# VisualComputingInstitute/diffusion-e2e-ft

Measured on AMD Instinct MI355X. Metric: images/sec (768x768, 1-step UNet fwd) full path: VAE encode + SD-v2 UNet @t=999 + VAE decode, higher is better.
Workload: dtype f16

## Files before the change

### diffusion-e2e-ft_amd/_lib.py

```python
import ctypes as C
import os

import torch

from . import build as _build

_LIB = None

F32, F16, BF16 = 0, 1, 2
_DT = {torch.float32: F32, torch.float16: F16, torch.bfloat16: BF16}


def dtype_id(dt):
    try:
        return _DT[dt]
    except KeyError:
        raise TypeError("libe2eft supports float32/float16/bfloat16, got %s" % dt)


class ConvDesc(C.Structure):
    _fields_ = [(n, C.c_int32) for n in (
        "dtype", "batch", "hin", "win", "hl", "wl", "c1", "ldx1", "c2", "ldx2", "kh", "kw", "stride", "pad_t", "pad_l",
        "hout", "wout", "cout", "ldo", "ldr", "ldw")] + [("alpha", C.c_float)]


class GemmDesc(C.Structure):
    _fields_ = ([(n, C.c_int32) for n in ("dtype", "m", "n", "k", "lda", "ldw", "ldo", "ldr", "nzo", "nzi")]
                + [(n, C.c_int64) for n in ("sa_o", "sa_i", "sw_o", "sw_i", "so_o", "so_i", "sr_o", "sr_i")]
                + [("bias_along_m", C.c_int32), ("alpha", C.c_float)])


class GroupNormDesc(C.Structure):
    _fields_ = [(n, C.c_int32) for n in ("dtype", "batch", "hw", "c1", "ldx1", "c2", "ldx2", "groups", "ldy", "silu")] + [
        ("eps", C.c_float)]


class AttnDesc(C.Structure):
    _fields_ = [(n, C.c_int32) for n in ("dtype", "batch", "heads", "nq", "nk_seg", "kv_nseg", "kv_bmod", "ldq", "ldk", "ldv",
                                          "ldo")] + [("scale", C.c_float)]


class NormalEvalDesc(C.Structure):
    _fields_ = [(n, C.c_int32) for n in ("batch", "height", "width", "reserved")] + [
        ("pred_stride", C.c_int64 * 4), ("gt_stride", C.c_int64 * 4), ("mask_stride", C.c_int64 * 3)]


class D2ntDesc(C.Structure):
    _fields_ = [(n, C.c_int32) for n in ("batch", "height", "width", "refine", "out_format")] + [("depth_scale", C.c_float)]


D2NT_F32, D2NT_U16, D2NT_U8 = range(3)


class HypersimDesc(C.Structure):
    _fields_ = [(n, C.c_int32) for n in ("batch", "height", "width", "color_dtype", "distance_dtype", "depth_format")] + [
        ("focal", C.c_double), ("scale_numerator", C.c_double)]


HYPERSIM_DEPTH_U16, HYPERSIM_DEPTH_F32 = range(2)
HYPERSIM_RECORD = 16


class DepthGtDesc(C.Structure):
    _fields_ = ([(n, C.c_int32) for n in ("batch", "h0", "w0", "raw_dtype")] + [("divisor", C.c_double)]
                + [(n, C.c_int32) for n in ("inf_to_zero", "crop_top", "crop_left", "crop_h", "crop_w")] + [("min_depth", C.c_float), ("max_depth", C.c_float)]
                + [(n, C.c_int32) for n in ("win_y0", "win_y1", "win_x0", "win_x1", "use_ext_mask")])


GT_U16, GT_I32, GT_F32 = range(3)


class NormalGtDesc(C.Structure):
    _fields_ = [(n, C.c_int32) for n in ("batch", "height", "width", "raw_dtype")]


NORMAL_GT_U8, NORMAL_GT_F32 = range(2)


class DsineRgbDesc(C.Structure):
    _fields_ = [(n, C.c_int32) for n in ("batch", "height", "width", "out_layout")]


class DiffusionDesc(C.Structure):
    _fields_ = [(n, C.c_int32) for n in ("dtype", "dtype_out", "prediction", "rows", "hw", "c", "batch", "ldx0", "ldn", "ldy", "n_timesteps")]


DIFFUSION_ADD_NOISE, DIFFUSION_VELOCITY = range(2)
PREDICTION_TYPES = {"epsilon": 0, "v_prediction": 1}


RGB_HWC, RGB_CHW = range(2)
DSINE_RGB_WS_INTS = 6


OPT_PERSISTENT, OPT_PERSISTENT_GRID, OPT_NARROW_CONV, OPT_NARROW_MFMA, OPT_IGEMM_GENERAL_OPERANDS, OPT_IGEMM2_WAVES, OPT_PATCH_CONV, OPT_THIN_INPUT_CONV, OPT_FUSED_NORM, OPT_ATTN_DMA, OPT_UPCONV_PHASES, OPT_PATCH_CONV_2X2, OPT_PERSISTENT_MIN_QROUNDS, OPT_GN_APPLY_ITERS, OPT_F32_SPLIT, OPT_F32_SPLIT_ATTN, OPT_PATCH_MFMA = range(17)

_P = C.c_void_p
_I = C.c_int32
_L = C.c_int64
_F = C.c_float
_Z = C.c_size_t

SIGNATURES = {
    "e2eft_version": (_I, []),
    "e2eft_last_error": (C.c_char_p, []),
    "e2eft_build_id": (C.c_char_p, []),
    "e2eft_set_option": (_I, [_I, _I]),
    "e2eft_get_option": (_I, [_I]),
    "e2eft_conv2d_fwd": (_I, [C.POINTER(ConvDesc), _P, _P, _P, _P, _P, _P, _P, _P]),
    "e2eft_gemm": (_I, [C.POINTER(GemmDesc), _P, _P, _P, _P, _P, _P]),
    "e2eft_conv2d_fwd_gnstats": (_I, [C.POINTER(ConvDesc), _P, _P, _P, _P, _P, _P, _P, _P, _Z, C.POINTER(C.c_int32), _P]),
    "e2eft_conv2d_splitk_workspace_bytes": (_Z, [C.POINTER(ConvDesc)]),
    "e2eft_conv2d_fwd_splitk": (_I, [C.POINTER(ConvDesc), _P, _P, _P, _P, _P, _P, _P, _P, _Z, _P]),
    "e2eft_gemm_gnstats": (_I, [C.POINTER(GemmDesc), _P, _P, _P, _P, _P, _I, _P, _Z, C.POINTER(C.c_int32), _P]),
    "e2eft_groupnorm_fwd_pre": (_I, [C.POINTER(GroupNormDesc), _P, _P, _P, _P, _P, _P, _I, _P, _I, _P, _Z, _P]),
    "e2eft_groupnorm_coeff_offset": (_Z, [C.POINTER(GroupNormDesc)]),
    "e2eft_groupnorm_fwd_stats": (_I, [C.POINTER(GroupNormDesc), _P, _P, _P, _P, _I, _P, _I, _P, _Z, _P]),
    "e2eft_conv2d_fwd_normed_supported": (_I, [C.POINTER(ConvDesc)]),
    "e2eft_upconv2x_fwd_supported": (_I, [C.POINTER(ConvDesc)]),
    "e2eft_upconv2x_fwd": (_I, [C.POINTER(ConvDesc), _P, _P, _P, _P, _P, _Z, C.POINTER(C.c_int32), _P]),
    "e2eft_groupnorm_fwd_split": (_I, [C.POINTER(GroupNormDesc), _P, _P, _P, _P, _I, _P, _P, _I, _P, _Z, _P]),
    "e2eft_f32_split_weight": (_I, [_P, _L, _I, _P, _P, _P]),
    "e2eft_f32_split2_cat": (_I, [_P, _I, _I, _P, _I, _I, _L, _P, _I, _P, _P]),
    "e2eft_f32_split2": (_I, [_P, _L, _I, _I, _P, _I, _P, _P]),
    "e2eft_f32_split2_cols": (_I, [_P, _I, _I, _P, _I, _I, _L, _P, _I, _P, _P]),
    "e2eft_f32_split_wgrad_finish": (_I, [_P, _P, _P, _L, _I, _I, _P, _P, _P, _P]),
    "e2eft_conv2d_fwd_f32split_supported": (_I, [C.POINTER(ConvDesc)]),
    "e2eft_conv2d_fwd_f32split": (_I, [C.POINTER(ConvDesc), _P, _P, _P, _P, _P, _P, _P, _P, _Z, C.POINTER(C.c_int32), _P]),
    "e2eft_upconv2x_fwd_f32split_supported": (_I, [C.POINTER(ConvDesc)]),
    "e2eft_upconv2x_fwd_f32split": (_I, [C.POINTER(ConvDesc), _P, _P, _P, _P, _P, _P, _P, _Z, C.POINTER(C.c_int32), _P]),
    "e2eft_gemm_f32split_supported": (_I, [C.POINTER(GemmDesc)]),
    "e2eft_attn_f32split_supported": (_I, [C.POINTER(AttnDesc), _I]),
    "e2eft_gemm_f32split": (_I, [C.POINTER(GemmDesc), _P, _P, _P, _P, _P, _P, _P, _P]),
    "e2eft_conv2d_fwd_normed": (_I, [C.POINTER(ConvDesc), _P, _P, _P, _I, _P, _P, _P, _P, _P, _P, _Z, C.POINTER(C.c_int32), _P]),
    "e2eft_groupnorm_workspace_bytes": (_Z, [C.POINTER(GroupNormDesc)]),
    "e2eft_groupnorm_fwd": (_I, [C.POINTER(GroupNormDesc), _P, _P, _P, _P, _P, _P, _Z, _P]),
    "e2eft_layernorm_fwd": (_I, [_I, _L, _I, _I, _I, _F, _P, _P, _P, _P, _P]),
    "e2eft_geglu_fwd": (_I, [_I, _L, _I, _I, _I, _P, _P, _P]),
    "e2eft_softmax_rows": (_I, [_I, _L, _I, _L, _F, _P, _P]),
    "e2eft_softmax_rows_causal": (_I, [_I, _L, _I, _L, _F, _I, _P, _P]),
    "e2eft_attn_fwd": (_I, [C.POINTER(AttnDesc), _P, _P, _P, _P, _P]),
    "e2eft_attn_fwd_lse": (_I, [C.POINTER(AttnDesc), _P, _P, _P, _P, _P, _P]),
    "e2eft_attn512_workspace_bytes": (_Z, [C.POINTER(AttnDesc)]),
    "e2eft_attn512_fwd": (_I, [C.POINTER(AttnDesc), _P, _P, _P, _P, _P, _Z, _P]),
    "e2eft_attn_bwd_workspace_bytes": (_Z, [C.POINTER(AttnDesc)]),
    "e2eft_attn_bwd": (_I, [C.POINTER(AttnDesc), _P, _P, _P, _P, _P, _I, _P, _P, _I, _P, _I, _P, _I, _P, _Z, _P]),
    "e2eft_nchw_to_nhwc": (_I, [_I, _I, _I, _I, _I, _I, _I, _F, _F, _P, _P, _P]),
    "e2eft_nhwc_to_nchw": (_I, [_I, _I, _I, _I, _I, _I, _F, _F, _P, _P, _P]),
    "e2eft_copy_scale": (_I, [_I, _L, _I, _I, _I, _F, _F, _P, _P, _P]),
    "e2eft_add": (_I, [_I, _L, _I, _I, _I, _I, _P, _P, _P, _P]),
    "e2eft_timestep_embedding": (_I, [_I, _I, _I, _P, _P, _P]),
    "e2eft_silu": (_I, [_I, _L, _P, _P, _P]),
    "e2eft_depth_head": (_I, [_I, _I, _L, _I, _I, _P, _P, _P]),
    "e2eft_normal_head": (_I, [_I, _I, _I, _I, _I, _I, _F, _P, _P, _P]),
    "e2eft_ssi_loss_workspace_bytes": (_Z, [_I]),
    "e2eft_ssi_loss_fwd": (_I, [_I, _I, _P, _P, _P, _P, _P, _P, _Z, _P]),
    "e2eft_angular_loss_workspace_bytes": (_Z, [_I]),
    "e2eft_angular_loss_fwd": (_I, [_I, _I, _P, _P, _P, _P, _P, _Z, _P]),
    "e2eft_conv2d_dgrad": (_I, [C.POINTER(ConvDesc), _P, _I, _I, _P, _I, _P, _I, _P]),
    "e2eft_conv2d_wgrad_workspace_bytes": (_Z, [C.POINTER(ConvDesc), _I]),
    "e2eft_conv2d_wgrad": (_I, [C.POINTER(ConvDesc), _P, _I, _P, _P, _P, _Z, C.POINTER(C.c_int32), _P]),
    "e2eft_conv2d_im2col_t": (_I, [C.POINTER(ConvDesc), _P, _P, _P, _L, _P]),
    "e2eft_transpose": (_I, [_I, _I, _L, _I, _L, _L, _L, _L, _L, _P, _P, _P]),
    "e2eft_colsum_workspace_bytes": (_Z, [_I, _L, _I]),
    "e2eft_colsum": (_I, [_I, _I, _L, _I, _L, _F, _P, _P, _P, _Z, _P]),
    "e2eft_upsample_nearest_bwd": (_I, [_I, _I, _I, _I, _I, _I, _I, _I, _I, _P, _P, _P]),
    "e2eft_groupnorm_bwd_workspace_bytes": (_Z, [C.POINTER(GroupNormDesc)]),
    "e2eft_groupnorm_bwd": (_I, [C.POINTER(GroupNormDesc), _P, _P, _P, _P, _P, _I, _P, _I, _P, _P, _P, _P, _Z, _P]),
    "e2eft_groupnorm_bwd_add": (_I, [C.POINTER(GroupNormDesc), _P, _P, _P, _P, _P, _I, _P, _I, _P, _I, _P, _P, _P, _P, _Z, _P]),
    "e2eft_layernorm_bwd_workspace_bytes": (_Z, [_L, _I]),
    "e2eft_layernorm_bwd": (_I, [_I, _L, _I, _I, _I, _I, _F, _P, _P, _P, _P, _P, _P, _Z, _P]),
    "e2eft_geglu_bwd": (_I, [_I, _L, _I, _I, _I, _I, _P, _P, _P, _P]),
    "e2eft_softmax_bwd_rows": (_I, [_I, _L, _I, _L, _F, _P, _P, _P]),
    "e2eft_silu_bwd": (_I, [_I, _L, _P, _P, _P, _P]),
    "e2eft_depth_head_bwd": (_I, [_I, _I, _L, _I, _I, _I, _I, _P, _P, _P, _P]),
    "e2eft_normal_head_bwd": (_I, [_I, _I, _I, _I, _I, _I, _I, _I, _F, _P, _P, _P, _P]),
    "e2eft_ssi_loss_bwd_workspace_bytes": (_Z, [_I]),
    "e2eft_ssi_loss_bwd": (_I, [_I, _I, _P, _P, _P, _P, _P, _P, _P, _P, _Z, _P]),
# ... 118 lines not shown
```

### diffusion-e2e-ft_amd/csrc/api.hip

```cpp
#include "common.h"
#include <atomic>

namespace e2eft {

static thread_local char g_err[512] = "";

char* err_buf() { return g_err; }

int fail(int code, const char* fmt, ...) {
    va_list ap;
    va_start(ap, fmt);
    vsnprintf(g_err, sizeof(g_err), fmt, ap);
    va_end(ap);
    return code;
}

int check_launch(const char* what) {
    hipError_t e = hipGetLastError();
    if (e != hipSuccess) return fail(E2EFT_ERR_LAUNCH, "%s: launch failed: %s", what, hipGetErrorString(e));
    return E2EFT_OK;
}

static std::atomic<int> g_cus_of_device[64];
int device_cus() {
    int dev = 0;
    if (hipGetDevice(&dev) != hipSuccess || dev < 0 || dev >= 64) return 0;
    int n = g_cus_of_device[dev].load(std::memory_order_relaxed);
    if (n == 0) {
        if (hipDeviceGetAttribute(&n, hipDeviceAttributeMultiprocessorCount, dev) != hipSuccess || n < 8) return 0;
        n &= ~7;
        g_cus_of_device[dev].store(n, std::memory_order_relaxed);
    }
    return n;
}

static thread_local char g_tag[96] = "";
void tag_kernel(const char* fmt, ...) {
    va_list ap;
    va_start(ap, fmt);
    vsnprintf(g_tag, sizeof(g_tag), fmt, ap);
    va_end(ap);
}
const char* last_tag() { return g_tag; }

static std::atomic<int> g_opt[E2EFT_OPT_COUNT] = {{1}, {0}, {1}, {1}, {0}, {0}, {1}, {1}, {1}, {1}, {1}, {1}, {2}, {0}, {1}, {0}, {0}};

int option(int key) { return g_opt[key].load(std::memory_order_relaxed); }

}

extern "C" int e2eft_set_option(int32_t key, int32_t value) {
    using namespace e2eft;
    E2EFT_REQUIRE(key >= 0 && key < E2EFT_OPT_COUNT, "set_option: unknown key %d", key);
    bool ok = value == 0 || value == 1;
    if (key == E2EFT_OPT_PERSISTENT_GRID) ok = value == 0 || (value >= 8 && value % 8 == 0 && value <= 4096);
    if (key == E2EFT_OPT_IGEMM2_WAVES) ok = value == 0 || value == 4 || value == 8;
    if (key == E2EFT_OPT_PERSISTENT_MIN_QROUNDS) ok = value >= 1 && value <= 64;
    if (key == E2EFT_OPT_GN_APPLY_ITERS) ok = value >= 0 && value <= 16;
    if (key == E2EFT_OPT_PATCH_MFMA) ok = value >= 0 && value <= 2;
    E2EFT_REQUIRE(ok, "set_option: value %d out of range for key %d", value, key);
    g_opt[key].store(value, std::memory_order_relaxed);
    return E2EFT_OK;
}
extern "C" int e2eft_get_option(int32_t key) { return key >= 0 && key < E2EFT_OPT_COUNT ? e2eft::option(key) : -1; }

extern "C" const char* e2eft_debug_last_kernel(void) { return e2eft::last_tag(); }

extern "C" int e2eft_version(void) { return E2EFT_VERSION; }
#ifndef E2EFT_BUILD_ID
#define E2EFT_BUILD_ID "unstamped"
#endif
static const char k_build_id[] = "E2EFT_BUILD_ID=" E2EFT_BUILD_ID;
extern "C" const char* e2eft_build_id(void) { return k_build_id + 15; }
extern "C" const char* e2eft_last_error(void) { return e2eft::err_buf(); }
```

### diffusion-e2e-ft_amd/csrc/igemm5.hip

```cpp
#include "igemm.h"
#include <atomic>
#include <type_traits>

namespace e2eft {

namespace pers {
constexpr int BM = 256, BN = 128, NW = 8;
constexpr int A_STAGE = BM * 128, B_STAGE = BN * 128, STAGE = A_STAGE + B_STAGE;
constexpr int RING = 3 * STAGE;
constexpr int DEP = NW * 64 * 3 * 4;
constexpr int ROWTAB = BM * 16;
constexpr int LDS = RING + DEP + ROWTAB;
}

#ifdef E2EFT_STAMPS
static __device__ long long g_stamps5[512 * 32 * 8];
#define STAMP5(t, i) do { if (threadIdx.x == 0 && (t) < 32 && blockIdx.x < 512) g_stamps5[(blockIdx.x * 32 + (t)) * 8 + (i)] = __builtin_readcyclecounter(); } while (0)
#else
#define STAMP5(t, i) do { } while (0)
#endif

template <typename T, int MODE, bool RES, bool F32O = false>
__global__ __launch_bounds__(512) void igemm5_kernel(const IgemmParams p, const int total_tiles) {
    using namespace pers;
    static_assert(!F32O || (RES && std::is_same<T, f16>::value), "fp32 output: the fp32-window epilogue, f16 split operands");
    __shared__ __attribute__((aligned(16))) char smem[LDS];
    constexpr int EPC = 8;
    constexpr int BK = 64;
    constexpr int RSTEP = 8 * NW;
    typedef float f2 __attribute__((ext_vector_type(2)));

    const int tid = threadIdx.x;
    const int lane = tid & 63;
    const int wave = __builtin_amdgcn_readfirstlane(tid >> 6);
    const int wm = wave >> 1, wn = wave & 1;
    const int l31 = lane & 31, h = lane >> 5;
    const int nblk = p.mtiles * p.ntiles;
    const int nk = p.K / BK;

    const int nslots = (int)gridDim.x >> 3, xcd = (int)blockIdx.x & 7, slot = (int)blockIdx.x >> 3;
    const int q8 = total_tiles >> 3, r8 = total_tiles & 7;
    const int cbeg = xcd < r8 ? xcd * (q8 + 1) : r8 * (q8 + 1) + (xcd - r8) * q8;
    const int cend = cbeg + (xcd < r8 ? q8 + 1 : q8);
    int u_dma = cbeg + slot;
    if (u_dma >= cend) return;

    const int lrow = 8 * wave + (lane >> 3);
    const int jc = (lane & 7) ^ ((lrow >> 1) & 7);
    const bool plain_taps = MODE == 1 && p.zins <= 1 && p.hl == p.hin && p.wl == p.win;
    const bool half_res = MODE == 1 && (p.zins == 2 || (p.zins <= 1 && p.hl == 2 * p.hin && p.wl == 2 * p.win));

    unsigned int off1[4], off2[4];
    unsigned int cur_a[4], cur_b[2];
    unsigned int base1[4], base2[4];
    int a_iy0[4], a_ix0[4], brel[4];
    int tile_c = 0, ky = 0, kx = 0;
    int d_m0 = 0, d_n0 = 0, d_zo = 0, d_zi = 0;
    bool dma_done = false;
    __amdgpu_buffer_rsrc_t rs1, rs2, rsw, rsa;

    int d_b0 = 0;
    auto tile_coords = [&](const int u) {
        int z = 0, lid = u;
        if (nblk != total_tiles) { z = fast_div(u, nblk); lid = u - z * nblk; }
        int mt = lid, nt = 0;
        if (p.ntiles > 1) { mt = fast_div(lid, p.ntiles); nt = lid - mt * p.ntiles; }
        d_m0 = mt * BM; d_n0 = nt * BN;
        d_zo = 0; d_zi = z;
        if (p.nzi > 1 && z > 0) { d_zo = fast_div(z, p.nzi); d_zi = z - d_zo * p.nzi; }
        else if (p.nzi == 1) { d_zo = z; d_zi = 0; }
        if (MODE == 1) d_b0 = fast_div(d_m0, p.hout * p.wout);
    };
    auto fill_rowtab = [&]() {
        if (MODE == 1 && tid < BM) {
            const int hw = p.hout * p.wout;
            const int m = d_m0 + tid;
            const int b = fast_div(m, hw);
            const int rem = m - b * hw;
            const int oy = fast_div(rem, p.wout), ox = rem - oy * p.wout;
            int iy0 = oy * p.stride - p.pad_t, ix0 = ox * p.stride - p.pad_l;
            if (F32O && m >= p.M) iy0 = -0x4000;
            const u32x4 v = {(unsigned)(b - d_b0), (unsigned)iy0, (unsigned)ix0, (unsigned)(((b - d_b0) * p.hin + iy0) * p.win + ix0)};
            const unsigned addr = (unsigned)(RING + DEP) + (unsigned)tid * 16u;
            asm volatile("ds_write_b128 %0, %1" :: "v"(addr), "v"(v) : "memory");
        }
    };
    auto finish_setup = [&]() {
        const T* X1 = (const T*)p.x1 + d_zo * p.sa_o + d_zi * p.sa_i;
        const T* W = (const T*)p.w + d_zo * p.sw_o + d_zi * p.sw_i;
        const T* b1;
        const T* b2 = (const T*)p.x2;
        if (MODE == 0) {
            b1 = X1 + (long)d_m0 * p.ldx1;
#pragma unroll
            for (int i = 0; i < 4; ++i) cur_a[i] = ((F32O && d_m0 + lrow + RSTEP * i >= p.M) ? SRD_OOB : (unsigned)((lrow + RSTEP * i) * p.ldx1 + jc * EPC) * (unsigned)sizeof(T)) - 128u;
        } else {
            b1 = X1 + (long)d_b0 * p.hin * p.win * p.ldx1;
            if (b2) b2 += (long)d_b0 * p.hin * p.win * p.ldx2;
            u32x4 rt[4];
#pragma unroll
            for (int i = 0; i < 4; ++i) {
                const unsigned addr = (unsigned)(RING + DEP) + (unsigned)(lrow + RSTEP * i) * 16u;
                asm volatile("ds_read_b128 %0, %1" : "=v"(rt[i]) : "v"(addr) : "memory");
            }
            asm volatile("s_waitcnt lgkmcnt(0)" : "+v"(rt[0]), "+v"(rt[1]), "+v"(rt[2]), "+v"(rt[3]) :: "memory");
#pragma unroll
            for (int i = 0; i < 4; ++i) {
                brel[i] = (int)rt[i][0]; a_iy0[i] = (int)rt[i][1]; a_ix0[i] = (int)rt[i][2];
                cur_a[i] = 0;
                if (plain_taps) {
                    base1[i] = (rt[i][3] * (unsigned)p.ldx1 + (unsigned)(jc * EPC)) * (unsigned)sizeof(T);
                    base2[i] = (rt[i][3] * (unsigned)p.ldx2 + (unsigned)(jc * EPC)) * (unsigned)sizeof(T);
                }
            }
        }
        rs1 = whole_range_rsrc(b1);
        rs2 = whole_range_rsrc((b2 ? b2 : b1));
        rsw = whole_range_rsrc((W + (long)d_n0 * p.ldw));
        rsa = rs1;
// ... 26 lines not shown
                off1[i] = ok ? (pix * (unsigned)p.ldx1 + (unsigned)(jc * EPC)) * (unsigned)sizeof(T) : SRD_OOB;
                off2[i] = ok ? (pix * (unsigned)p.ldx2 + (unsigned)(jc * EPC)) * (unsigned)sizeof(T) : SRD_OOB;
            }
            return;
        }
#pragma unroll
        for (int i = 0; i < 4; ++i) {
            const int iy = a_iy0[i] + ky, ix = a_ix0[i] + kx;
            bool ok = (unsigned)iy < (unsigned)p.hl && (unsigned)ix < (unsigned)p.wl;
            int sy = iy, sx = ix;
            if (p.zins > 1) {
                ok = ok && (iy % p.zins == 0) && (ix % p.zins == 0);
                sy = iy / p.zins; sx = ix / p.zins;
            } else {
                if (p.hl != p.hin) sy = min((int)floorf(iy * p.up_sh), p.hin - 1);
                if (p.wl != p.win) sx = min((int)floorf(ix * p.up_sw), p.win - 1);
            }
            const unsigned pix = (unsigned)((brel[i] * p.hin + sy) * p.win + sx);
            off1[i] = ok ? (pix * (unsigned)p.ldx1 + (unsigned)(jc * EPC)) * (unsigned)sizeof(T) : SRD_OOB;
            off2[i] = ok ? (pix * (unsigned)p.ldx2 + (unsigned)(jc * EPC)) * (unsigned)sizeof(T) : SRD_OOB;
        }
    };
#ifdef E2EFT_STAMPS
    bool fire_a = true;
#endif
    auto advance = [&]() {
#ifdef E2EFT_STAMPS
        fire_a = !(p.debug_flags & 1) && !((p.debug_flags & 2) && kx != 0) && !((p.debug_flags & 4) && (kx != 0 || ky != 0));
#endif
        if (MODE == 0) {
            if constexpr (F32O) {
                const unsigned back = tile_c == p.split_c ? (unsigned)p.split_c * 2u : 0u;
                tile_c += BK;
#pragma unroll
                for (int i = 0; i < 4; ++i) cur_a[i] += 128u - back;
            } else {
#pragma unroll
                for (int i = 0; i < 4; ++i) cur_a[i] += 128u;
            }
        } else {
            if (F32O && tile_c == p.split_c) {
#pragma unroll
                for (int i = 0; i < 4; ++i) cur_a[i] = off1[i];
            } else if (tile_c == 0) {
                retap();
#pragma unroll
                for (int i = 0; i < 4; ++i) cur_a[i] = off1[i];
                rsa = rs1;
            } else if (tile_c == p.c1) {
#pragma unroll
                for (int i = 0; i < 4; ++i) cur_a[i] = off2[i];
                rsa = rs2;
            } else {
#pragma unroll
                for (int i = 0; i < 4; ++i) cur_a[i] += 128u;
            }
            tile_c += BK;
            if (tile_c >= p.cin) {
                tile_c = 0;
                if (++kx == p.kw) { kx = 0; ++ky; }
            }
        }
        cur_b[0] += 128u;
        cur_b[1] += 128u;
    };
    int s_cur = 0, s_nxt = STAGE, s_dst = 2 * STAGE;
    auto rotate = [&]() { const int t = s_cur; s_cur = s_nxt; s_nxt = s_dst; s_dst = t; };
    auto fire = [&](const int stage, auto piece_c) {
        constexpr int Q = decltype(piece_c)::value;
        char* sa = smem + stage + wave * 1024;
#ifdef E2EFT_STAMPS
        if (Q < 4 && !fire_a) return;
#endif
        if constexpr (Q < 4) __builtin_amdgcn_raw_ptr_buffer_load_lds(rsa, (lds_ptr_t)(sa + Q * (RSTEP * 128)), 16, cur_a[Q], 0, 0, 0);
        else __builtin_amdgcn_raw_ptr_buffer_load_lds(rsw, (lds_ptr_t)(sa + A_STAGE + (Q - 4) * (RSTEP * 128)), 16, cur_b[Q - 4], 0, 0, 0);
    };
    auto fire_all = [&](const int stage) {
        fire(stage, IConst<0>{}); fire(stage, IConst<1>{}); fire(stage, IConst<2>{}); fire(stage, IConst<3>{});
        fire(stage, IConst<4>{}); fire(stage, IConst<5>{});
    };

    int tseq = 0;
    (void)tseq;
    floatx16 acc[2][2];
    const int sw = (l31 >> 1) & 7;
    int aofs[4], bofs[4];
#pragma unroll
    for (int g = 0; g < 4; ++g) {
        const int chunk = g * 2 + h;
        aofs[g] = (wm * 64 + l31) * 128 + ((chunk ^ sw) * 16);
        bofs[g] = A_STAGE + (wn * 64 + l31) * 128 + ((chunk ^ sw) * 16);
    }
    auto mma_group = [&](const u32x4& a0, const u32x4& a1, const u32x4& b0, const u32x4& b1) {
        acc[0][0] = Mma32x32x16<T>::run(a0, b0, acc[0][0]);
        acc[0][1] = Mma32x32x16<T>::run(a0, b1, acc[0][1]);
        acc[1][0] = Mma32x32x16<T>::run(a1, b0, acc[1][0]);
        acc[1][1] = Mma32x32x16<T>::run(a1, b1, acc[1][1]);
    };

    const int er = lane >> 3, ec = lane & 7;
    const T* __restrict__ bias = (const T*)p.bias;
    const T* __restrict__ rowadd = (const T*)p.rowadd;
    constexpr bool has_res = RES && !F32O;
    const bool has_ra = rowadd != nullptr, stats = p.gn_partial != nullptr;
    Vec16<T> pre_res[4], pre_bias, pre_ra;
    T col_bias[2], col_ra[2];
    long c_orow = 0, c_rrow = 0;
    int c_m0 = 0, c_n0 = 0, c_img = 0, c_ncl = 0;
    int c_mb = 0, c_seg0 = 0;
    bool c_colok = false;

    const int npre = F32O ? 0 : has_res ? 4 + (bias ? 1 : 0) + (has_ra ? 1 : 0) : 2 * ((bias ? 1 : 0) + (has_ra ? 1 : 0));
    bool nxt = false;
    long zoff_o = 0;
    auto enter_tile = [&]() {
        c_m0 = d_m0; c_n0 = d_n0;
        zoff_o = d_zo * p.so_o + d_zi * p.so_i;
        const long zoff_r = d_zo * p.sr_o + d_zi * p.sr_i;
        c_colok = c_n0 + wn * 64 + ec * 8 < p.N;
        c_ncl = c_colok ? c_n0 + wn * 64 + ec * 8 : c_n0;
        c_img = has_ra ? fast_div(c_m0, p.rows_per_img) : 0;
        const int m = c_m0 + wm * 64 + er;
        c_mb = c_m0 + wm * 64;
        c_seg0 = p.out_seg > 0 ? fast_div(c_mb, p.out_seg) : 0;
        c_orow = ((long)m + (long)c_seg0 * p.out_seg) * p.ldo + c_ncl;
        c_rrow = zoff_r + (long)m * p.ldr + c_ncl;
        nxt = u_dma + nslots < cend;
        if (nxt) tile_coords(u_dma + nslots);
    };
    auto ktile = [&](auto kind_c, const int nextwait) {
        constexpr int KIND = decltype(kind_c)::value;
        if (KIND == 0 || KIND == 3 || (KIND == 2 && !dma_done)) advance();
        const int sc = s_cur, sd = s_dst;
        u32x4 a0[3], a1[3], b0[3], b1[3];
        auto rd = [&](auto gc, auto slotc) {
            constexpr int g = decltype(gc)::value, slot = decltype(slotc)::value;
            a0[slot] = *reinterpret_cast<const u32x4*>(smem + sc + aofs[g]);
            a1[slot] = *reinterpret_cast<const u32x4*>(smem + sc + aofs[g] + 32 * 128);
            b0[slot] = *reinterpret_cast<const u32x4*>(smem + sc + bofs[g]);
            b1[slot] = *reinterpret_cast<const u32x4*>(smem + sc + bofs[g] + 32 * 128);
        };
        rd(IConst<0>{}, IConst<0>{});
        rd(IConst<1>{}, IConst<1>{});
        __builtin_amdgcn_sched_barrier(0);
        rd(IConst<2>{}, IConst<2>{});
        if constexpr (KIND != 1) { fire(sd, IConst<0>{}); fire(sd, IConst<1>{}); }
        __builtin_amdgcn_sched_barrier(0);
        if constexpr (KIND == 3) {
            const floatx16 z = {0.f, 0.f, 0.f, 0.f, 0.f, 0.f, 0.f, 0.f, 0.f, 0.f, 0.f, 0.f, 0.f, 0.f, 0.f, 0.f};
            acc[0][0] = Mma32x32x16<T>::run(a0[0], b0[0], z);
            acc[0][1] = Mma32x32x16<T>::run(a0[0], b1[0], z);
            acc[1][0] = Mma32x32x16<T>::run(a1[0], b0[0], z);
            acc[1][1] = Mma32x32x16<T>::run(a1[0], b1[0], z);
        } else {
            mma_group(a0[0], a1[0], b0[0], b1[0]);
        }
        __builtin_amdgcn_sched_barrier(0);
        if constexpr (KIND == 3) enter_tile();
        if constexpr (KIND == 1) {
            if constexpr (F32O) {
            } else if (has_res) {
#pragma unroll
                for (int s = 0; s < 4; ++s) pre_res[s] = ld16((const T*)p.residual + c_rrow + (long)(s * 8) * p.ldr);
                if (bias) pre_bias = ld16(bias + c_ncl);
                if (has_ra) pre_ra = ld16(rowadd + (long)c_img * p.N + c_ncl);
            } else {
                const int cA = c_n0 + wn * 64 + l31, cB = cA + 32;
                const int nA = cA < p.N ? cA : c_n0, nB = cB < p.N ? cB : c_n0;
                if (bias) { col_bias[0] = bias[nA]; col_bias[1] = bias[nB]; }
                if (has_ra) { col_ra[0] = rowadd[(long)c_img * p.N + nA]; col_ra[1] = rowadd[(long)c_img * p.N + nB]; }
            }
            u_dma += nslots;
            if (nxt) {
                finish_setup();
                advance();
            } else {
                dma_done = true;
#pragma unroll
                for (int i = 0; i < 4; ++i) cur_a[i] = SRD_OOB;
                cur_b[0] = cur_b[1] = SRD_OOB;
            }
            __builtin_amdgcn_sched_barrier(0);
            fire(sd, IConst<0>{}); fire(sd, IConst<1>{});
        }
        rd(IConst<3>{}, IConst<0>{});
        fire(sd, IConst<2>{}); fire(sd, IConst<3>{});
        __builtin_amdgcn_sched_barrier(0);
        mma_group(a0[1], a1[1], b0[1], b1[1]);
        __builtin_amdgcn_sched_barrier(0);
        fire(sd, IConst<4>{}); fire(sd, IConst<5>{});
        if constexpr (KIND == 3) {
            if (nxt) fill_rowtab();
        }
        __builtin_amdgcn_sched_barrier(0);
        if (nextwait == 2) asm volatile("s_waitcnt vmcnt(6) lgkmcnt(0)" ::: "memory");
        else if (nextwait == 3) {
            if (npre == 0) asm volatile("s_waitcnt vmcnt(6) lgkmcnt(0)" ::: "memory");
            else if (npre == 1) asm volatile("s_waitcnt vmcnt(7) lgkmcnt(0)" ::: "memory");
            else if (npre == 2) asm volatile("s_waitcnt vmcnt(8) lgkmcnt(0)" ::: "memory");
            else if (npre == 4) asm volatile("s_waitcnt vmcnt(10) lgkmcnt(0)" ::: "memory");
            else if (npre == 5) asm volatile("s_waitcnt vmcnt(11) lgkmcnt(0)" ::: "memory");
            else asm volatile("s_waitcnt vmcnt(12) lgkmcnt(0)" ::: "memory");
        } else asm volatile("s_waitcnt lgkmcnt(0)" ::: "memory");
        __builtin_amdgcn_s_barrier();
        asm volatile("" ::: "memory");
        __builtin_amdgcn_sched_barrier(0);
        mma_group(a0[2], a1[2], b0[2], b1[2]);
        mma_group(a0[0], a1[0], b0[0], b1[0]);
        asm volatile("" ::: "memory");
        rotate();
    };

    auto epi_rows_left = [&]() -> int { return F32O ? p.M - (c_m0 + wm * 64 + er) : 0x40000000; };
    auto epi_rofs = [&](const int r) -> long {
        if (p.out_seg <= 0) return (long)r;
        return (long)r + (long)(fast_div(c_mb + r, p.out_seg) - c_seg0) * p.out_seg;
    };
    constexpr int EPI_DEP = RING;
    constexpr bool EPI_M16 = false;
    auto epi_srow = [&](const int s) -> int { return 8 * s; };
#define EPI_STAMP(i) STAMP5(tseq, i)
#include "igemm_persistent_epilogue.inc"
#undef EPI_STAMP
    const float al_f32 = F32O ? p.alpha * (p.alpha_dev ? *p.alpha_dev : 1.f) * (p.alpha_dev2 ? *p.alpha_dev2 : 1.f) : 0.f;
    tile_coords(u_dma);
    fill_rowtab();
    __syncthreads();
    finish_setup();
    advance(); fire_all(s_cur);
    advance(); fire_all(s_nxt);
    asm volatile("s_waitcnt vmcnt(6)" ::: "memory");
    __builtin_amdgcn_s_barrier();
    asm volatile("" ::: "memory");
    bool first = true;
    for (;;) {
        STAMP5(tseq, 0);
        ktile(IConst<3>{}, first ? 2 : 0);
        for (int kt = 1; kt < nk - 2; ++kt) ktile(IConst<0>{}, 2);
        STAMP5(tseq, 1);
        ktile(IConst<1>{}, 3);
        STAMP5(tseq, 4);
        ktile(IConst<2>{}, 0);
        STAMP5(tseq, 2);
        if constexpr (F32O) epilogue_f32(s_dst, al_f32);
        else if constexpr (RES) epilogue(s_dst, zoff_o);
        else epilogue_packed(s_dst, zoff_o);
        STAMP5(tseq, 3);
        ++tseq;
        asm volatile("s_waitcnt lgkmcnt(0)" ::: "memory");
        __builtin_amdgcn_s_barrier();
        asm volatile("" ::: "memory");
        if (stats) { const int img = c_m0 / p.rows_per_img; combine(img, (c_m0 - img * p.rows_per_img) / BM, c_n0); }
        STAMP5(tseq - 1, 7);
        if (dma_done) break;
        first = false;
    }
}

static std::atomic<long> g_pers_launches{0};

#ifdef E2EFT_STAMPS
extern int g_debug_flags5;
#endif

template <typename T, int MODE> static int launch5(IgemmParams& p, int nz, int total, int grid, hipStream_t s) {
    if constexpr (std::is_same<T, f16>::value) {
        if (p.split_c > 0) {
            hipLaunchKernelGGL((igemm5_kernel<f16, MODE, true, true>), dim3(grid), dim3(512), 0, s, p, total);
            tag_kernel("igemm5_kernel<_Float16, %d, true, f32split>", MODE);
            return check_launch("igemm5");
        }
    }
    if (p.residual) hipLaunchKernelGGL((igemm5_kernel<T, MODE, true>), dim3(grid), dim3(512), 0, s, p, total);
    else hipLaunchKernelGGL((igemm5_kernel<T, MODE, false>), dim3(grid), dim3(512), 0, s, p, total);
    tag_kernel("igemm5_kernel<%s, %d, %s>", std::is_same<T, f16>::value ? "_Float16" : "__bf16", MODE, p.residual ? "true" : "false");
    return check_launch("igemm5");
}

bool igemm_persistent_eligible(int dtype, int mode, const IgemmParams& p, int nz, TilePlan& t) {
    using namespace pers;
    if (!option(E2EFT_OPT_PERSISTENT)) return false;
    if (dtype != E2EFT_F16 && dtype != E2EFT_BF16) return false;
    if (p.ksplit_taps > 0 || p.bias_along_m) return false;
    if (p.split_c > 0 && (dtype != E2EFT_F16 || nz != 1 || p.x2 || p.rowadd || p.split_c % 64 != 0 || p.cin != 3 * p.split_c || p.c1 != p.cin ||
                          (mode == 0 && p.K != 3 * p.split_c))) return false;
    if ((p.M % BM != 0 && !(p.split_c > 0 && p.out_seg == 0 && p.M > BM)) || p.K % 64 != 0 || p.K / 64 < 3) return false;
    if (!vec_epilogue_ok(p)) return false;
    if (p.rowadd && (!al16(p.rowadd) || (p.rows_per_img % BM != 0 && p.rows_per_img < p.M))) return false;
    if (nz > 1 && (p.so_o % 8 != 0 || p.so_i % 8 != 0 || p.sr_o % 8 != 0 || p.sr_i % 8 != 0)) return false;
    if (p.out_seg != 0 && (p.out_seg < 16 || p.out_seg % 16 != 0 || nz != 1 || p.residual || p.M % p.out_seg != 0)) return false;
    if ((mode != 0 && (p.cin % 64 != 0 || p.c1 % 64 != 0)) || !fast_operands_in_range(mode, p, 2)) return false;
    const int cus = persistent_grid();
    if (!plan_tiles(p, nz, BM, BN, cus, (long)option(E2EFT_OPT_PERSISTENT_MIN_QROUNDS) * cus, t)) return false;
    return !p.gn_partial || (nz == 1 && p.rows_per_img % BM == 0 && p.M % p.rows_per_img == 0);
}

int launch_igemm_persistent(int dtype, int mode, IgemmParams& p, int nz, hipStream_t s) {
    TilePlan t;
    if (!igemm_persistent_eligible(dtype, mode, p, nz, t)) return -1;
    apply_plan(p, t);
    g_pers_launches.fetch_add(1, std::memory_order_relaxed);
#ifdef E2EFT_STAMPS
    p.debug_flags = g_debug_flags5;
#endif
    if (dtype == E2EFT_F16) return mode ? launch5<f16, 1>(p, nz, (int)t.total, t.grid, s) : launch5<f16, 0>(p, nz, (int)t.total, t.grid, s);
    return mode ? launch5<bf16, 1>(p, nz, (int)t.total, t.grid, s) : launch5<bf16, 0>(p, nz, (int)t.total, t.grid, s);
}

}

#ifdef E2EFT_STAMPS
namespace e2eft { int g_debug_flags5 = 0; }
extern "C" void e2eft_debug_set_flags5(int f) { e2eft::g_debug_flags5 = f; }
extern "C" int e2eft_debug_read_stamps5(long long* host, int nworkgroups) {
    return (int)hipMemcpyFromSymbol(host, HIP_SYMBOL(e2eft::g_stamps5), (size_t)nworkgroups * 32 * 8 * sizeof(long long));
}
#endif
extern "C" long e2eft_debug_persistent_launches(void) { return e2eft::g_pers_launches.load(); }
```

### include/e2eft.h

```cpp
#ifndef E2EFT_H
#define E2EFT_H

#include <stddef.h>
#include <stdint.h>

#ifdef __cplusplus
extern "C" {
#endif
#pragma GCC visibility push(default)

#define E2EFT_VERSION 119

enum {
    E2EFT_OK = 0,
    E2EFT_ERR_BAD_ARG = 1,
    E2EFT_ERR_WORKSPACE = 2,
    E2EFT_ERR_LAUNCH = 3,
    E2EFT_ERR_UNSUPPORTED = 4,
};

enum { E2EFT_F32 = 0, E2EFT_F16 = 1, E2EFT_BF16 = 2 };

int e2eft_version(void);
const char* e2eft_last_error(void);
const char* e2eft_build_id(void);

enum {
    E2EFT_OPT_PERSISTENT = 0,
    E2EFT_OPT_PERSISTENT_GRID = 1,
    E2EFT_OPT_NARROW_CONV = 2,
    E2EFT_OPT_NARROW_MFMA = 3,
    E2EFT_OPT_IGEMM_GENERAL_OPERANDS = 4,
    E2EFT_OPT_IGEMM2_WAVES = 5,
    E2EFT_OPT_PATCH_CONV = 6,
    E2EFT_OPT_THIN_INPUT_CONV = 7,
    E2EFT_OPT_FUSED_NORM = 8,
    E2EFT_OPT_ATTN_DMA = 9,
    E2EFT_OPT_UPCONV_PHASES = 10,
    E2EFT_OPT_PATCH_CONV_2X2 = 11,
    E2EFT_OPT_PERSISTENT_MIN_QROUNDS = 12,
    E2EFT_OPT_GN_APPLY_ITERS = 13,
    E2EFT_OPT_F32_SPLIT = 14,
    E2EFT_OPT_F32_SPLIT_ATTN = 15,
    E2EFT_OPT_PATCH_MFMA = 16,
    E2EFT_OPT_COUNT = 17
};
int e2eft_set_option(int32_t key, int32_t value);
int e2eft_get_option(int32_t key);

typedef struct E2eftConvDesc {
    int32_t dtype;
    int32_t batch, hin, win, hl, wl;
    int32_t c1, ldx1;
    int32_t c2, ldx2;
    int32_t kh, kw, stride;
    int32_t pad_t, pad_l;
    int32_t hout, wout;
    int32_t cout, ldo;
    int32_t ldr;
    int32_t ldw;
    float alpha;
} E2eftConvDesc;

int e2eft_conv2d_fwd(const E2eftConvDesc* d, const void* x1, const void* x2, const void* w,
                     const void* bias ,
                     const void* rowadd ,
                     const void* residual , void* out, void* stream);

typedef struct E2eftGemmDesc {
    int32_t dtype;
    int32_t m, n, k;
    int32_t lda, ldw, ldo, ldr;
    int32_t nzo, nzi;
    int64_t sa_o, sa_i, sw_o, sw_i, so_o, so_i, sr_o, sr_i;
    int32_t bias_along_m;
    float alpha;
} E2eftGemmDesc;

int e2eft_gemm(const E2eftGemmDesc* d, const void* a, const void* w, const void* bias, const void* residual,
               void* out, void* stream);

int e2eft_conv2d_fwd_gnstats(const E2eftConvDesc* d, const void* x1, const void* x2, const void* w, const void* bias,
                             const void* rowadd, const void* residual, void* out, float* gn_partial,
                             size_t gn_partial_bytes, int32_t* slab_rows, void* stream);
int e2eft_conv2d_fwd_normed_supported(const E2eftConvDesc* d);
int e2eft_upconv2x_fwd_supported(const E2eftConvDesc* d);
int e2eft_upconv2x_fwd(const E2eftConvDesc* d, const void* x, const void* w_phase, const void* bias, void* out, float* gn_partial,
                       size_t gn_partial_bytes, int32_t* slab_rows, void* stream);

int e2eft_f32_split2(const float* x, int64_t pixels, int32_t c, int32_t ldx, void* planes, int32_t ldp, float* scale, void* stream);
int e2eft_f32_split_weight(const float* w, int64_t rows, int32_t c, void* w_split, float* scale, void* stream);
int e2eft_f32_split2_cat(const float* x1, int32_t c1, int32_t ldx1, const float* x2, int32_t c2, int32_t ldx2, int64_t pixels, void* planes, int32_t ldp,
                         float* scale, void* stream);
int e2eft_f32_split2_cols(const float* x1, int32_t c1, int32_t ldx1, const float* x2, int32_t c2, int32_t ldx2, int64_t pixels, void* planes, int32_t ldp,
                          float* colscale, void* stream);
int e2eft_f32_split_wgrad_finish(const float* t0, const float* t1, const float* t2, int64_t cout, int32_t taps, int32_t cin, const float* inv_dy, const float* inv_x,
                                 float* out, void* stream);
int e2eft_conv2d_fwd_f32split_supported(const E2eftConvDesc* d);
int e2eft_conv2d_fwd_f32split(const E2eftConvDesc* d, const void* planes, const float* scale, const void* w_split, const float* w_inv_scale, const float* bias,
                              const float* residual, float* out, float* gn_partial, size_t gn_partial_bytes, int32_t* slab_rows, void* stream);
int e2eft_upconv2x_fwd_f32split_supported(const E2eftConvDesc* d);
int e2eft_upconv2x_fwd_f32split(const E2eftConvDesc* d, const void* planes, const float* scale, const void* w_phase_split, const float* w_inv_scale,
                                const float* bias, float* out, float* gn_partial, size_t gn_partial_bytes, int32_t* slab_rows, void* stream);
int e2eft_gemm_f32split_supported(const E2eftGemmDesc* d);
int e2eft_gemm_f32split(const E2eftGemmDesc* d, const void* planes, const float* scale, const void* w_split, const float* w_inv_scale, const float* bias,
                        const float* residual, float* out, void* stream);
int e2eft_conv2d_fwd_normed(const E2eftConvDesc* d, const void* x1, const float* coeff, const void* beta, int32_t silu, const void* w,
                            const void* bias, const void* rowadd, const void* residual, void* out, float* gn_partial,
                            size_t gn_partial_bytes, int32_t* slab_rows, void* stream);
size_t e2eft_conv2d_splitk_workspace_bytes(const E2eftConvDesc* d);
int e2eft_conv2d_fwd_splitk(const E2eftConvDesc* d, const void* x1, const void* x2, const void* w, const void* bias,
                            const void* rowadd, const void* residual, void* out, void* workspace, size_t ws_bytes, void* stream);
int e2eft_gemm_gnstats(const E2eftGemmDesc* d, const void* a, const void* w, const void* bias, const void* residual,
                       void* out, int32_t rows_per_image, float* gn_partial, size_t gn_partial_bytes,
                       int32_t* slab_rows, void* stream);

typedef struct E2eftGroupNormDesc {
    int32_t dtype;
    int32_t batch, hw;
    int32_t c1, ldx1, c2, ldx2;
    int32_t groups;
    int32_t ldy;
    int32_t silu;
    float eps;
} E2eftGroupNormDesc;

size_t e2eft_groupnorm_workspace_bytes(const E2eftGroupNormDesc* d);
int e2eft_groupnorm_fwd(const E2eftGroupNormDesc* d, const void* x1, const void* x2, const void* gamma,
// ... 248 lines not shown
```

### include/e2eft_debug.h

```cpp
#ifndef E2EFT_DEBUG_H
#define E2EFT_DEBUG_H
#ifdef __cplusplus
extern "C" {
#endif
#pragma GCC visibility push(default)

const char* e2eft_debug_last_kernel(void);
long e2eft_debug_patch_launches(void);
long e2eft_debug_persistent_launches(void);
long e2eft_debug_thin_launches(void);

int e2eft_debug_read_stamps(long long* host, int nworkgroups);
int e2eft_debug_read_stamps_rt(long long* host, int nworkgroups);
int e2eft_debug_read_stamps5(long long* host, int nworkgroups);
void e2eft_debug_set_flags5(int flags);

#pragma GCC visibility pop
#ifdef __cplusplus
}
#endif
#endif
```

Measured before the change: 91.10.

## Add 16x16x32 MFMA variant of persistent implicit-GEMM kernel with shape-based selection

Adds an M16 template form of the persistent igemm5 kernel that computes each wave's 64x64 tile with a 4x4 grid of 16x16x32 MFMAs instead of 2x2 32x32x16 MFMAs. This needs new LDS fragment addressing, a new k-tile schedule (ktile16) and a different epilogue row mapping. A heuristic table enables it by default for conv modes and for some f16 GEMM shapes, with an option to force either form. The aim is better MFMA throughput and latency for these shapes, at the cost of more accumulator registers and a larger, riskier code path.

```diff
diff --git a/diffusion-e2e-ft_amd/_lib.py b/diffusion-e2e-ft_amd/_lib.py
--- a/diffusion-e2e-ft_amd/_lib.py
+++ b/diffusion-e2e-ft_amd/_lib.py
@@ -93,7 +93,7 @@
 DSINE_RGB_WS_INTS = 6
 
 
-OPT_PERSISTENT, OPT_PERSISTENT_GRID, OPT_NARROW_CONV, OPT_NARROW_MFMA, OPT_IGEMM_GENERAL_OPERANDS, OPT_IGEMM2_WAVES, OPT_PATCH_CONV, OPT_THIN_INPUT_CONV, OPT_FUSED_NORM, OPT_ATTN_DMA, OPT_UPCONV_PHASES, OPT_PATCH_CONV_2X2, OPT_PERSISTENT_MIN_QROUNDS, OPT_GN_APPLY_ITERS, OPT_F32_SPLIT, OPT_F32_SPLIT_ATTN, OPT_PATCH_MFMA = range(17)
+OPT_PERSISTENT, OPT_PERSISTENT_GRID, OPT_NARROW_CONV, OPT_NARROW_MFMA, OPT_IGEMM_GENERAL_OPERANDS, OPT_IGEMM2_WAVES, OPT_PATCH_CONV, OPT_THIN_INPUT_CONV, OPT_FUSED_NORM, OPT_ATTN_DMA, OPT_UPCONV_PHASES, OPT_PATCH_CONV_2X2, OPT_PERSISTENT_MIN_QROUNDS, OPT_GN_APPLY_ITERS, OPT_F32_SPLIT, OPT_F32_SPLIT_ATTN, OPT_PATCH_MFMA, OPT_PERSISTENT_MFMA = range(18)
 
 _P = C.c_void_p
 _I = C.c_int32
diff --git a/diffusion-e2e-ft_amd/csrc/api.hip b/diffusion-e2e-ft_amd/csrc/api.hip
--- a/diffusion-e2e-ft_amd/csrc/api.hip
+++ b/diffusion-e2e-ft_amd/csrc/api.hip
@@ -43,7 +43,7 @@
 }
 const char* last_tag() { return g_tag; }
 
-static std::atomic<int> g_opt[E2EFT_OPT_COUNT] = {{1}, {0}, {1}, {1}, {0}, {0}, {1}, {1}, {1}, {1}, {1}, {1}, {2}, {0}, {1}, {0}, {0}};
+static std::atomic<int> g_opt[E2EFT_OPT_COUNT] = {{1}, {0}, {1}, {1}, {0}, {0}, {1}, {1}, {1}, {1}, {1}, {1}, {2}, {0}, {1}, {0}, {0}, {0}};
 
 int option(int key) { return g_opt[key].load(std::memory_order_relaxed); }
 
@@ -57,7 +57,7 @@
     if (key == E2EFT_OPT_IGEMM2_WAVES) ok = value == 0 || value == 4 || value == 8;
     if (key == E2EFT_OPT_PERSISTENT_MIN_QROUNDS) ok = value >= 1 && value <= 64;
     if (key == E2EFT_OPT_GN_APPLY_ITERS) ok = value >= 0 && value <= 16;
-    if (key == E2EFT_OPT_PATCH_MFMA) ok = value >= 0 && value <= 2;
+    if (key == E2EFT_OPT_PATCH_MFMA || key == E2EFT_OPT_PERSISTENT_MFMA) ok = value >= 0 && value <= 2;
     E2EFT_REQUIRE(ok, "set_option: value %d out of range for key %d", value, key);
     g_opt[key].store(value, std::memory_order_relaxed);
     return E2EFT_OK;
diff --git a/diffusion-e2e-ft_amd/csrc/igemm5.hip b/diffusion-e2e-ft_amd/csrc/igemm5.hip
--- a/diffusion-e2e-ft_amd/csrc/igemm5.hip
+++ b/diffusion-e2e-ft_amd/csrc/igemm5.hip
@@ -20,10 +20,10 @@
 #define STAMP5(t, i) do { } while (0)
 #endif
 
-template <typename T, int MODE, bool RES, bool F32O = false>
+template <typename T, int MODE, bool RES, bool F32O = false, bool M16 = false>
 __global__ __launch_bounds__(512) void igemm5_kernel(const IgemmParams p, const int total_tiles) {
     using namespace pers;
-    static_assert(!F32O || (RES && std::is_same<T, f16>::value), "fp32 output: the fp32-window epilogue, f16 split operands");
+    static_assert(!F32O || (RES && !M16 && std::is_same<T, f16>::value), "fp32 output: the fp32-window epilogue, f16 split operands, the 32x32x16 form");
     __shared__ __attribute__((aligned(16))) char smem[LDS];
     constexpr int EPC = 8;
     constexpr int BK = 64;
@@ -35,6 +35,7 @@
     const int wave = __builtin_amdgcn_readfirstlane(tid >> 6);
     const int wm = wave >> 1, wn = wave & 1;
     const int l31 = lane & 31, h = lane >> 5;
+    const int r15 = lane & 15, q4 = lane >> 4;
     const int nblk = p.mtiles * p.ntiles;
     const int nk = p.K / BK;
 
@@ -227,7 +228,7 @@
 
     int tseq = 0;
     (void)tseq;
-    floatx16 acc[2][2];
+    std::conditional_t<M16, floatx4[4][4], floatx16[2][2]> acc;
     const int sw = (l31 >> 1) & 7;
     int aofs[4], bofs[4];
 #pragma unroll
@@ -236,11 +237,25 @@
         aofs[g] = (wm * 64 + l31) * 128 + ((chunk ^ sw) * 16);
         bofs[g] = A_STAGE + (wn * 64 + l31) * 128 + ((chunk ^ sw) * 16);
     }
+    const int a16 = (wm * 64 + r15) * 128 + ((q4 ^ (r15 >> 1)) << 4);
+    const int b16 = A_STAGE + (wn * 64 + r15) * 128 + ((q4 ^ (r15 >> 1)) << 4);
     auto mma_group = [&](const u32x4& a0, const u32x4& a1, const u32x4& b0, const u32x4& b1) {
-        acc[0][0] = Mma32x32x16<T>::run(a0, b0, acc[0][0]);
-        acc[0][1] = Mma32x32x16<T>::run(a0, b1, acc[0][1]);
-        acc[1][0] = Mma32x32x16<T>::run(a1, b0, acc[1][0]);
-        acc[1][1] = Mma32x32x16<T>::run(a1, b1, acc[1][1]);
+        if constexpr (!M16) {
+            acc[0][0] = Mma32x32x16<T>::run(a0, b0, acc[0][0]);
+            acc[0][1] = Mma32x32x16<T>::run(a0, b1, acc[0][1]);
+            acc[1][0] = Mma32x32x16<T>::run(a1, b0, acc[1][0]);
+            acc[1][1] = Mma32x32x16<T>::run(a1, b1, acc[1][1]);
+        }
+    };
+    auto mma_rows = [&](auto i0c, const u32x4& a0, const u32x4& a1, const u32x4 (&b)[4], auto zc) {
+        constexpr int i0 = decltype(i0c)::value;
+        if constexpr (M16) {
+            const floatx4 z = {0.f, 0.f, 0.f, 0.f};
+#pragma unroll
+            for (int j = 0; j < 4; ++j) acc[i0][j] = Mma16x16x32<T>::run(a0, b[j], decltype(zc)::value ? z : acc[i0][j]);
+#pragma unroll
+            for (int j = 0; j < 4; ++j) acc[i0 + 1][j] = Mma16x16x32<T>::run(a1, b[j], decltype(zc)::value ? z : acc[i0 + 1][j]);
+        }
     };
 
     const int er = lane >> 3, ec = lane & 7;
@@ -249,13 +264,16 @@
     constexpr bool has_res = RES && !F32O;
     const bool has_ra = rowadd != nullptr, stats = p.gn_partial != nullptr;
     Vec16<T> pre_res[4], pre_bias, pre_ra;
-    T col_bias[2], col_ra[2];
+    T col_bias[M16 ? 4 : 2], col_ra[M16 ? 4 : 2];
     long c_orow = 0, c_rrow = 0;
     int c_m0 = 0, c_n0 = 0, c_img = 0, c_ncl = 0;
     int c_mb = 0, c_seg0 = 0;
     bool c_colok = false;
 
-    const int npre = F32O ? 0 : has_res ? 4 + (bias ? 1 : 0) + (has_ra ? 1 : 0) : 2 * ((bias ? 1 : 0) + (has_ra ? 1 : 0));
+    const int npre = F32O ? 0 : has_res ? 4 + (bias ? 1 : 0) + (has_ra ? 1 : 0) : (M16 ? 4 : 2) * ((bias ? 1 : 0) + (has_ra ? 1 : 0));
+    const int er_row = (M16 && RES) ? 4 * (er >> 1) + (er & 1) : er;
+    constexpr bool EPI_M16 = M16;
+    auto epi_srow = [&](const int s) -> int { return M16 ? 16 * (s >> 1) + 2 * (s & 1) : 8 * s; };
     bool nxt = false;
     long zoff_o = 0;
     auto enter_tile = [&]() {
@@ -265,7 +283,7 @@
         c_colok = c_n0 + wn * 64 + ec * 8 < p.N;
         c_ncl = c_colok ? c_n0 + wn * 64 + ec * 8 : c_n0;
         c_img = has_ra ? fast_div(c_m0, p.rows_per_img) : 0;
-        const int m = c_m0 + wm * 64 + er;
+        const int m = c_m0 + wm * 64 + er_row;
         c_mb = c_m0 + wm * 64;
         c_seg0 = p.out_seg > 0 ? fast_div(c_mb, p.out_seg) : 0;
         c_orow = ((long)m + (long)c_seg0 * p.out_seg) * p.ldo + c_ncl;
@@ -291,7 +309,8 @@
         rd(IConst<2>{}, IConst<2>{});
         if constexpr (KIND != 1) { fire(sd, IConst<0>{}); fire(sd, IConst<1>{}); }
         __builtin_amdgcn_sched_barrier(0);
-        if constexpr (KIND == 3) {
+        if constexpr (M16) {
+        } else if constexpr (KIND == 3) {
             const floatx16 z = {0.f, 0.f, 0.f, 0.f, 0.f, 0.f, 0.f, 0.f, 0.f, 0.f, 0.f, 0.f, 0.f, 0.f, 0.f, 0.f};
             acc[0][0] = Mma32x32x16<T>::run(a0[0], b0[0], z);
             acc[0][1] = Mma32x32x16<T>::run(a0[0], b1[0], z);
@@ -355,6 +374,84 @@
         asm volatile("" ::: "memory");
         rotate();
     };
+    auto ktile16 = [&](auto kind_c, const int nextwait) {
+        constexpr int KIND = decltype(kind_c)::value;
+        if (KIND == 0 || KIND == 3 || (KIND == 2 && !dma_done)) advance();
+        const int sc = s_cur, sd = s_dst;
+        u32x4 fa[6], fb[2][4];
+        auto rd_a = [&](auto ksc, auto ic, auto slotc) {
+            constexpr int ks = decltype(ksc)::value, i = decltype(ic)::value, sl = decltype(slotc)::value;
+            fa[sl] = *reinterpret_cast<const u32x4*>(smem + ((sc + a16) ^ (ks << 6)) + i * 2048);
+        };
+        auto rd_b = [&](auto ksc) {
+            constexpr int ks = decltype(ksc)::value;
+#pragma unroll
+            for (int j = 0; j < 4; ++j) fb[ks][j] = *reinterpret_cast<const u32x4*>(smem + ((sc + b16) ^ (ks << 6)) + j * 2048);
+        };
+        rd_a(IConst<0>{}, IConst<0>{}, IConst<0>{}); rd_a(IConst<0>{}, IConst<1>{}, IConst<1>{});
+        rd_a(IConst<0>{}, IConst<2>{}, IConst<2>{}); rd_a(IConst<0>{}, IConst<3>{}, IConst<3>{});
+        rd_b(IConst<0>{});
+        __builtin_amdgcn_sched_barrier(0);
+        rd_b(IConst<1>{});
+        if constexpr (KIND != 1) { fire(sd, IConst<0>{}); fire(sd, IConst<1>{}); }
+        __builtin_amdgcn_sched_barrier(0);
+        mma_rows(IConst<0>{}, fa[0], fa[1], fb[0], std::bool_constant<KIND == 3>{});
+        __builtin_amdgcn_sched_barrier(0);
+        if constexpr (KIND == 3) enter_tile();
+        if constexpr (KIND == 1) {
+            if (has_res) {
+#pragma unroll
+                for (int s = 0; s < 4; ++s) pre_res[s] = ld16((const T*)p.residual + c_rrow + (long)epi_srow(s) * p.ldr);
+                if (bias) pre_bias = ld16(bias + c_ncl);
+                if (has_ra) pre_ra = ld16(rowadd + (long)c_img * p.N + c_ncl);
+            } else {
+#pragma unroll
+                for (int j = 0; j < 4; ++j) {
+                    const int cj = c_n0 + wn * 64 + 16 * j + r15, nj = cj < p.N ? cj : c_n0;
+                    if (bias) col_bias[j] = bias[nj];
+                    if (has_ra) col_ra[j] = rowadd[(long)c_img * p.N + nj];
+                }
+            }
+            u_dma += nslots;
+            if (nxt) {
+                finish_setup();
+                advance();
+            } else {
+                dma_done = true;
+#pragma unroll
+                for (int i = 0; i < 4; ++i) cur_a[i] = SRD_OOB;
+                cur_b[0] = cur_b[1] = SRD_OOB;
+            }
+            __builtin_amdgcn_sched_barrier(0);
+            fire(sd, IConst<0>{}); fire(sd, IConst<1>{});
+        }
+        rd_a(IConst<1>{}, IConst<0>{}, IConst<0>{}); rd_a(IConst<1>{}, IConst<1>{}, IConst<1>{});
+        rd_a(IConst<1>{}, IConst<2>{}, IConst<4>{}); rd_a(IConst<1>{}, IConst<3>{}, IConst<5>{});
+        fire(sd, IConst<2>{}); fire(sd, IConst<3>{});
+        __builtin_amdgcn_sched_barrier(0);
+        mma_rows(IConst<2>{}, fa[2], fa[3], fb[0], std::bool_constant<KIND == 3>{});
+        __builtin_amdgcn_sched_barrier(0);
+        fire(sd, IConst<4>{}); fire(sd, IConst<5>{});
+        if constexpr (KIND == 3) {
+            if (nxt) fill_rowtab();
+        }
+        __builtin_amdgcn_sched_barrier(0);
+        if (nextwait == 2) asm volatile("s_waitcnt vmcnt(6) lgkmcnt(0)" ::: "memory");
+        else if (nextwait == 3) {
+            if (npre == 0) asm volatile("s_waitcnt vmcnt(6) lgkmcnt(0)" ::: "memory");
+            else if (npre == 4) asm volatile("s_waitcnt vmcnt(10) lgkmcnt(0)" ::: "memory");
+            else if (npre == 5) asm volatile("s_waitcnt vmcnt(11) lgkmcnt(0)" ::: "memory");
+            else if (npre == 6) asm volatile("s_waitcnt vmcnt(12) lgkmcnt(0)" ::: "memory");
+            else asm volatile("s_waitcnt vmcnt(14) lgkmcnt(0)" ::: "memory");
+        } else asm volatile("s_waitcnt lgkmcnt(0)" ::: "memory");
+        __builtin_amdgcn_s_barrier();
+        asm volatile("" ::: "memory");
+        __builtin_amdgcn_sched_barrier(0);
+        mma_rows(IConst<0>{}, fa[0], fa[1], fb[1], std::false_type{});
+        mma_rows(IConst<2>{}, fa[4], fa[5], fb[1], std::false_type{});
+        asm volatile("" ::: "memory");
+        rotate();
+    };
 
     auto epi_rows_left = [&]() -> int { return F32O ? p.M - (c_m0 + wm * 64 + er) : 0x40000000; };
     auto epi_rofs = [&](const int r) -> long {
@@ -362,8 +459,6 @@
         return (long)r + (long)(fast_div(c_mb + r, p.out_seg) - c_seg0) * p.out_seg;
     };
     constexpr int EPI_DEP = RING;
-    constexpr bool EPI_M16 = false;
-    auto epi_srow = [&](const int s) -> int { return 8 * s; };
 #define EPI_STAMP(i) STAMP5(tseq, i)
 #include "igemm_persistent_epilogue.inc"
 #undef EPI_STAMP
@@ -380,12 +475,21 @@
     bool first = true;
     for (;;) {
         STAMP5(tseq, 0);
+        if constexpr (M16) {
+            ktile16(IConst<3>{}, first ? 2 : 0);
+            for (int kt = 1; kt < nk - 2; ++kt) ktile16(IConst<0>{}, 2);
+            STAMP5(tseq, 1);
+            ktile16(IConst<1>{}, 3);
+            STAMP5(tseq, 4);
+            ktile16(IConst<2>{}, 0);
+        } else {
         ktile(IConst<3>{}, first ? 2 : 0);
         for (int kt = 1; kt < nk - 2; ++kt) ktile(IConst<0>{}, 2);
         STAMP5(tseq, 1);
         ktile(IConst<1>{}, 3);
         STAMP5(tseq, 4);
         ktile(IConst<2>{}, 0);
+        }
         STAMP5(tseq, 2);
         if constexpr (F32O) epilogue_f32(s_dst, al_f32);
         else if constexpr (RES) epilogue(s_dst, zoff_o);
@@ -408,6 +512,21 @@
 extern int g_debug_flags5;
 #endif
 
+static bool persistent_form16_table(int dtype, int mode, int K, int N, long M, int stride) {
+    (void)M; (void)stride;
+    if (dtype != E2EFT_F16 && dtype != E2EFT_BF16) return false;
+    if (mode != 0) return true;
+    return dtype == E2EFT_F16 && (N <= 320 || K >= 1280);
+}
+
+static bool persistent_form16(int dtype, int mode, const IgemmParams& p) {
+    if (p.split_c > 0) return false;
+    const int opt = option(E2EFT_OPT_PERSISTENT_MFMA);
+    if (opt == 1) return false;
+    if (opt == 2) return true;
+    return persistent_form16_table(dtype, mode, p.K, p.N, (long)p.M, mode ? p.stride : 1);
+}
+
 template <typename T, int MODE> static int launch5(IgemmParams& p, int nz, int total, int grid, hipStream_t s) {
     if constexpr (std::is_same<T, f16>::value) {
         if (p.split_c > 0) {
@@ -416,9 +535,16 @@
             return check_launch("igemm5");
         }
     }
+    const char* tn = std::is_same<T, f16>::value ? "_Float16" : "__bf16";
+    if (persistent_form16(std::is_same<T, f16>::value ? E2EFT_F16 : E2EFT_BF16, MODE, p)) {
+        if (p.residual) hipLaunchKernelGGL((igemm5_kernel<T, MODE, true, false, true>), dim3(grid), dim3(512), 0, s, p, total);
+        else hipLaunchKernelGGL((igemm5_kernel<T, MODE, false, false, true>), dim3(grid), dim3(512), 0, s, p, total);
+        tag_kernel("igemm5_kernel<%s, m16, %d, %s>", tn, MODE, p.residual ? "true" : "false");
+        return check_launch("igemm5");
+    }
     if (p.residual) hipLaunchKernelGGL((igemm5_kernel<T, MODE, true>), dim3(grid), dim3(512), 0, s, p, total);
     else hipLaunchKernelGGL((igemm5_kernel<T, MODE, false>), dim3(grid), dim3(512), 0, s, p, total);
-    tag_kernel("igemm5_kernel<%s, %d, %s>", std::is_same<T, f16>::value ? "_Float16" : "__bf16", MODE, p.residual ? "true" : "false");
+    tag_kernel("igemm5_kernel<%s, %d, %s>", tn, MODE, p.residual ? "true" : "false");
     return check_launch("igemm5");
 }
 
@@ -462,3 +588,6 @@
 }
 #endif
 extern "C" long e2eft_debug_persistent_launches(void) { return e2eft::g_pers_launches.load(); }
+extern "C" int e2eft_debug_persistent_form16(int dtype, int mode, int K, int N, long M, int stride) {
+    return e2eft::persistent_form16_table(dtype, mode, K, N, M, stride) ? 1 : 0;
+}
diff --git a/include/e2eft.h b/include/e2eft.h
--- a/include/e2eft.h
+++ b/include/e2eft.h
@@ -43,7 +43,8 @@
     E2EFT_OPT_F32_SPLIT = 14,
     E2EFT_OPT_F32_SPLIT_ATTN = 15,
     E2EFT_OPT_PATCH_MFMA = 16,
-    E2EFT_OPT_COUNT = 17
+    E2EFT_OPT_PERSISTENT_MFMA = 17,
+    E2EFT_OPT_COUNT = 18
 };
 int e2eft_set_option(int32_t key, int32_t value);
 int e2eft_get_option(int32_t key);
diff --git a/include/e2eft_debug.h b/include/e2eft_debug.h
--- a/include/e2eft_debug.h
+++ b/include/e2eft_debug.h
@@ -9,6 +9,7 @@
 long e2eft_debug_patch_launches(void);
 long e2eft_debug_persistent_launches(void);
 long e2eft_debug_thin_launches(void);
+int e2eft_debug_persistent_form16(int dtype, int mode, int K, int N, long M, int stride);
 
 int e2eft_debug_read_stamps(long long* host, int nworkgroups);
 int e2eft_debug_read_stamps_rt(long long* host, int nworkgroups);
```

New measurement: 91.42 (median of 6 runs). Within noise of the previous version (+0.3%).
